# evolbioinfo/pastml

Measured on AMD Instinct MI355X. Metric: ACR nodes*states*chars/sec (full marginal pass: P(t) + bottom-up + top-down + posteriors), higher is better.
Workload: dtype f64; 1 GPU; BASELINE config 4 shard: balanced tree, 1048576 tips (2097151 nodes), k=64 states, F81, 32 characters per GPU (32 in total), marginal (BU+TD+posteriors); tips=1048576, nodes=2097151, states=64, chars_per_gpu=32, chars_total=32, substitution_model=F81, collective=local

## Files before the change

### pastml_amd/csrc/pml_kernels_f81.h

```cpp
#pragma once
#include "pml_device.h"
#include "pml_schedule.h"

typedef unsigned char pml_jt;

struct PmlTree {
    int N;
    int n_roots;
    const int* parent;
    const int* first_child;
    const int* n_children;
    const double* dist;
    const int* post_rank;
    const unsigned char* kind;
};

struct PmlCols {
    int k, ks, W;
    int no_wide_lean;
    const u64* masks;
    const u64* masks_init;
    const double* pi;
    const double* active;
};
// ... 2045 lines not shown
    double te[2][2], ts[2][2];
    u64 tw[2][2][Q];
#pragma unroll
    for (int j = 0; j < 2; ++j) {
        const int ch = fc + (j < nc ? j : 0);
        const int code = j < nc ? unit_code(u.packed, j) : 0;
        ce[j] = L.E[ch];
        lane_words_issue<G, R>(L, c, ch, cw[j]);
        cs[j] = L.S[ch];
        cbe[j] = code == 1 ? L.be[ch] : 0;
        if (code == 1) {
            node_load_vec<G, R>(L, c, L.bu, ch, vv[j]);
        } else {
#pragma unroll
            for (int r = 0; r < R; ++r) vv[j][r] = 0.0;
        }
        const int cfc = j == 0 ? cfc0 : cfc1;
#pragma unroll
        for (int q = 0; q < 2; ++q) {
            te[j][q] = 0.0;
            ts[j][q] = 0.0;
#pragma unroll
            for (int x = 0; x < Q; ++x) tw[j][q][x] = 0ull;
            if (code >= 2 && q < code - 1) {
                te[j][q] = L.E[cfc + q];
                ts[j][q] = L.S[cfc + q];
                lane_words_issue<G, R>(L, c, cfc + q, tw[j][q]);
            }
        }
    }
    double prod[R];
#pragma unroll
    for (int r = 0; r < R; ++r) prod[r] = po[r] * (ls * L.ipi_r[r]);
#pragma unroll
    for (int j = 0; j < 2; ++j) {
        if (j < nc) {
            const int ch = fc + j;
            const int code = unit_code(u.packed, j);
            const double e = ce[j];
            unsigned cb[Q];
            lane_words_bits<G, R>(L, c, cw[j], cb);
            double mb[R], tdc[R], pc[R], lsc;
            bits_to_vec<R>(cb, mb);
            i64 xe, le;
            if (code == 0) {
                f81_finish_child<G, R>(L, c, prod, pe, ch, e, cs[j], 0, mb, false, mb, tdc, xe, pc, lsc, le, -1);
            } else if (code == 1) {
                double v[R];
#pragma unroll
                for (int r = 0; r < R; ++r) v[r] = vv[j][r];
                f81_finish_child<G, R>(L, c, prod, pe, ch, e, cs[j], cbe[j], v, false, mb, tdc, xe, pc, lsc, le, -1);
                if (st.td != nullptr) {
                    node_store_vec<G, R>(L, c, L.td, ch, tdc);
                    if (L.g == 0) L.te[ch] = xe;
                }
            } else {
                double v[R];
#pragma unroll
                for (int r = 0; r < R; ++r) v[r] = mb[r];
                double amin = 1.0;
                i64 bec = 0;
                unsigned tb[2][Q];
#pragma unroll
                for (int q = 0; q < 2; ++q) {
                    lane_words_bits<G, R>(L, c, tw[j][q], tb[q]);
                    if (q < code - 1) {
                        const double ta = (1.0 - te[j][q]) * ts[j][q];
                        double tmsg[R];
                        bits_select_vec<R>(tb[q], ta, te[j][q], tmsg);
                        amin *= ta;
#pragma unroll
                        for (int r = 0; r < R; ++r) v[r] *= tmsg[r];
                    }
                }
                if (!(amin >= 0x1p-190)) bec = lazy_rescale<G, R>(v);
                f81_finish_child<G, R>(L, c, prod, pe, ch, e, cs[j], bec, v, false, mb, tdc, xe, pc, lsc, le, -1);
                double prod2[R];
#pragma unroll
                for (int r = 0; r < R; ++r) prod2[r] = pc[r] * (lsc * L.ipi_r[r]);
                const int cfc = j == 0 ? cfc0 : cfc1;
#pragma unroll
                for (int q = 0; q < 2; ++q) {
                    if (q < code - 1) {
                        double mt[R], tdt[R], pt[R], lt;
                        bits_to_vec<R>(tb[q], mt);
                        i64 xt, et;
                        f81_finish_child<G, R>(L, c, prod2, le, cfc + q, te[j][q], ts[j][q], 0, mt, false, mt, tdt, xt, pt, lt, et, -1);
                    }
                }
            }
        }
    }
}

template <int G, int R, bool LEAN = false, bool SHAPES = false>
__device__ __forceinline__ void td_f81_unit(const LaneCtx<G, R>& L, const PmlTree& t, const PmlCols& c,
                                            const PmlState& st, const UnitRegs& u) {
    if (LEAN && G < 8 && c.W == 1 && unit_is_lean(u.packed)) {
        const int key = u.packed & (15 | (63 << 8));
        const int key0 = __builtin_amdgcn_readfirstlane(key);
        if (SHAPES && __ballot(key != key0) == 0ull) {
            switch (key0) {
                case PML_SHAPE_KEY(2, 1, 1): td_f81_unit_lean<G, R, 1, 1>(L, t, c, st, u); break;
                case PML_SHAPE_KEY(2, 3, 3): td_f81_unit_lean<G, R, 3, 3>(L, t, c, st, u); break;
                case PML_SHAPE_KEY(2, 1, 0): td_f81_unit_lean<G, R, 1, 0>(L, t, c, st, u); break;
                case PML_SHAPE_KEY(2, 0, 1): td_f81_unit_lean<G, R, 0, 1>(L, t, c, st, u); break;
                case PML_SHAPE_KEY(2, 1, 3): td_f81_unit_lean<G, R, 1, 3>(L, t, c, st, u); break;
                case PML_SHAPE_KEY(2, 3, 1): td_f81_unit_lean<G, R, 3, 1>(L, t, c, st, u); break;
                case PML_SHAPE_KEY(2, 0, 3): td_f81_unit_lean<G, R, 0, 3>(L, t, c, st, u); break;
                case PML_SHAPE_KEY(2, 3, 0): td_f81_unit_lean<G, R, 3, 0>(L, t, c, st, u); break;
                default: td_f81_unit_lean<G, R>(L, t, c, st, u); break;
            }
        } else {
            td_f81_unit_lean<G, R>(L, t, c, st, u);
        }
        return;
    }
    if (SHAPES && LEAN && G >= 2 && G < 8 && c.W == 1 && !c.no_wide_lean) {
        const bool poly = unit_is_lean_poly(u.packed);
        if (__ballot(!poly) == 0ull) {
            td_f81_unit_lean_poly<G, R>(L, t, c, st, u);
            return;
        }
    }
    if constexpr (G >= 32) {
        if (LEAN && c.W > 1 && !c.no_wide_lean && unit_is_lean(u.packed)) {
            const int cfc0 = __shfl(u.cfc, L.group_base, 64), cfc1 = __shfl(u.cfc, L.group_base + Gather<G>::GC, 64);
            td_f81_unit_lean_w<G, R>(L, t, c, st, u, cfc0, cfc1);
            return;
        }
    }
    if (Gather<G>::enabled && c.W == 1 && unit_is_fast<G>(u.packed)) {
        td_f81_unit_fast<G, R>(L, t, c, st, u);
        return;
    }
    const int p = u.n;

    double prod[R];
    i64 pe;
    f81_parent_prod<G, R>(L, c, p, prod, pe);
    double P = 0.0;
    bool have_P = false;
    const int fc = u.fc;
    int nc = unit_nc(u.packed);
    if (nc == 15) nc = t.n_children[p];
    for (int j = 0; j < nc; ++j) {
        const int ch = fc + j;
        const ChildDesc cd = unit_child<G>(t, u, j, ch);
        const int kd = cd.kind;
        const int slot = j < 2 ? j : -1;
        if (kd == PML_KIND_TIP) {
            f81_finish_tip<G, R>(L, c, prod, pe, P, have_P, ch, slot);
            continue;
        }
        const double e = L.E[ch];
        double mb[R], v[R], tdc[R], po[R], ls;
        node_mask_vec<G, R>(L, c, ch, mb);
        i64 xe, le;
        if (kd == PML_KIND_STORED) {
            node_load_vec<G, R>(L, c, L.bu, ch, v);
            f81_finish_child<G, R>(L, c, prod, pe, ch, e, L.S[ch], L.be[ch], v, false, mb, tdc, xe, po, ls, le, slot);
            if (st.td != nullptr) {
                node_store_vec<G, R>(L, c, L.td, ch, tdc);
                if (L.g == 0) L.te[ch] = xe;
            }
        } else {
            i64 bec;
            f81_cherry_vector<G, R>(L, t, c, st, ch, v, bec, false, cd.tips_known, cd.fc2, cd.nc2);
            const double s_child = L.S[ch];
            f81_finish_child<G, R>(L, c, prod, pe, ch, e, s_child, bec, v, false, mb, tdc, xe, po, ls, le, slot);
            double prod2[R];
#pragma unroll
            for (int r = 0; r < R; ++r) prod2[r] = po[r] * (ls * L.ipi_r[r]);
            const i64 pe2 = le;
            double P2 = 0.0;
            bool have_P2 = false;
            const int fc2 = cd.tips_known ? cd.fc2 : t.first_child[ch];
            const int nc2 = cd.tips_known ? cd.nc2 : t.n_children[ch];
            for (int q = 0; q < nc2; ++q)
                f81_finish_tip<G, R>(L, c, prod2, pe2, P2, have_P2, fc2 + q, (j < 2 && q < 2) ? 2 + 2 * j + q : -1);
        }
    }
}

struct TdStage {
    double* rows;
    double* sum;
    i64* exp;
    int* id;
    int* tid;
    int* tst;
};
__host__ __device__ __forceinline__ int td_stage_doubles(int uw, int ks, bool scalars) {
    return uw * 2 * ks + (scalars ? uw * 12 : 0) + uw * 5;
}

template <int G, int R>
__device__ __forceinline__ void td_stage_flush(const LaneCtx<G, R>& L, const PmlCols& c, const TdStage& S, bool tips) {
    typedef double dbl2 __attribute__((ext_vector_type(2)));
    constexpr int UW = 64 / G;
    wave_sync_lds();
    const int lane = threadIdx.x & 63;
    const int ppr = c.ks >> 1;
    for (int p = lane; p < UW * 2 * ppr; p += 64) {
        const int slot = p / ppr, piece = p - slot * ppr;
        const int node = S.id[slot];
        if (node >= 0) {
            const dbl2 v = *reinterpret_cast<const dbl2*>(S.rows + slot * c.ks + 2 * piece);
            __builtin_nontemporal_store(v, reinterpret_cast<dbl2*>(L.post + (size_t)(unsigned)node * c.ks + 2 * piece));
        }
    }
    for (int p = lane; tips && p < UW * 4 * ppr; p += 64) {
        const int slot = p / ppr, piece = p - slot * ppr;
        const int node = S.tid[slot];
        if (node >= 0) {
            const int s = S.tst[slot];
            dbl2 v;
            v.x = s == 2 * piece ? 1.0 : 0.0;
            v.y = s == 2 * piece + 1 ? 1.0 : 0.0;
            __builtin_nontemporal_store(v, reinterpret_cast<dbl2*>(L.post + (size_t)(unsigned)node * c.ks + 2 * piece));
        }
    }
    if (S.sum != nullptr) {
        for (int e = lane; e < UW * 6; e += 64) {
            const int u = e / 6, j = e - u * 6;
            if (j >= 2 && !tips) continue;
            const int node = j < 2 ? S.id[u * 2 + j] : S.tid[u * 4 + j - 2];
            if (node >= 0) {
                L.lhsum[node] = S.sum[e];
                L.lhe[node] = S.exp[e];
            }
        }
    }
    wave_sync_lds();
    for (int e = lane; e < UW * 2; e += 64) S.id[e] = -1;
    for (int e = lane; tips && e < UW * 4; e += 64) S.tid[e] = -1;
    wave_sync_lds();
}

template <int G, int R>
__global__ void __launch_bounds__(PML_BLOCK)
td_f81_kernel(PmlTree t, PmlCols c, PmlState st, const PmlUnit* __restrict__ units, int n_level, int stage) {
    extern __shared__ double td_stage[];
    constexpr int UW = 64 / G;
    const int wave = threadIdx.x >> 6;
    const int sub = (threadIdx.x & 63) / G;
    LaneCtx<G, R> L;
    lane_ctx_init<G, R>(L, t, c, st);
    TdStage S = {nullptr, nullptr, nullptr, nullptr, nullptr, nullptr};
    const bool staged = G <= PML_TD_STAGE_MAX_G && (stage & 1) && (c.ks & 1) == 0;
    if (staged) {
        const bool scalars = (stage & 2) != 0;
        double* base = td_stage + wave * td_stage_doubles(UW, c.ks, scalars);
        S.rows = base;
        base += UW * 2 * c.ks;
        if (scalars) {
            S.sum = base;
            S.exp = reinterpret_cast<i64*>(base + UW * 6);
            base += UW * 12;
        }
        S.id = reinterpret_cast<int*>(base);
        S.tid = S.id + UW * 2;
        S.tst = S.tid + UW * 4;
        L.srow = S.rows + sub * 2 * c.ks;
        L.sid = S.id + sub * 2;
        L.stid = S.tid + sub * 4;
        L.stst = S.tst + sub * 4;
        if (scalars) {
            L.ssum = S.sum + sub * 6;
            L.sexp = S.exp + sub * 6;
        }
        for (int e = threadIdx.x & 63; e < UW * 2; e += 64) S.id[e] = -1;
        for (int e = threadIdx.x & 63; e < UW * 4; e += 64) S.tid[e] = -1;
        wave_sync_lds();
    }
    const int stride = gridDim.x * PML_WAVES_PER_BLOCK * UW;
    int idx = (blockIdx.x * PML_WAVES_PER_BLOCK + wave) * UW + sub;
    UnitRegs cur = load_unit<G>(units, idx < n_level ? idx : 0, L.g);
    for (int base = idx - sub; base < n_level; base += stride) {
        const int nxt_idx = idx + stride;
        const UnitRegs nxt = load_unit<G>(units, nxt_idx < n_level ? nxt_idx : 0, L.g);
        if (idx < n_level) td_f81_unit<G, R, true>(L, t, c, st, cur);
        if (staged) td_stage_flush<G, R>(L, c, S, (stage & 4) != 0);
        cur = nxt;
        idx = nxt_idx;
    }
}


template <int G, int R>
__device__ __forceinline__ void td_f81_super_tips(const LaneCtx<G, R>& L, const PmlCols& c, const double (&prod3)[R],
                                                  i64 le, int cfc, const TipLane& tl, int jx) {
    constexpr int GC = Gather<G>::GC;
    double P3 = 0.0;
    bool have_P3 = false;
#pragma unroll
    for (int q = 0; q < 2; ++q) {
        const int ts = L.group_base + jx * GC + q;
        f81_finish_tip_word<G, R>(L, c, prod3, le, P3, have_P3, cfc + q, __shfl(tl.mask, ts, 64), __shfl(tl.e, ts, 64),
                                  __shfl(tl.s, ts, 64));
    }
}

template <int G, int R, bool LANES>
__device__ __forceinline__ void td_f81_super_unit(const LaneCtx<G, R>& L, const PmlTree& t, const PmlCols& c,
                                                  const PmlState& st, const SuperRegs& s, int j, double* ps_row) {
    const u64 kbits = state_bits(c.k);
    const int ch = s.fc + j;
    const UnitRegs u = super_child<G>(s, j, L.g);
    double prod[R];
    i64 pe;
    f81_parent_prod<G, R>(L, c, s.n, prod, pe);
    const double e = L.E[ch];
    const double s_child = L.S[ch];
    const i64 bec = L.be[ch];
    BuLoads<R> ld;
    ld.own = L.mask[(unsigned)ch];
    f81_gather_issue<G, R>(L, u, ld.cl, ld.tl);
    f81_gather_finish<G, R>(L, ld.cl, ld.tl);
    ld.own &= kbits;
    const bool all_ones = __all(c.k == G * R && ld.own == kbits && ld.cl.mask == kbits);
    BuResult<R> v;
    CherryKeep<R> ck;
    if (all_ones) bu_f81_marg_body<G, R, false, true, true>(L, t, c, st, u, ld, &v, false, true, &ck);
    else bu_f81_marg_body<G, R, false, false, true>(L, t, c, st, u, ld, &v, false, true, &ck);
    double prod2[R];
    i64 pe2;
    {
        double mb[R], tdc[R], po[R], ls;
        const bool full = ld.own == kbits;
        if (!full) clean_word_to_vec<G, R>(L, c, ld.own, mb);
        i64 xe;
        f81_finish_child<G, R>(L, c, prod, pe, ch, e, s_child, bec, v.v, full, mb, tdc, xe, po, ls, pe2);
        if (st.td != nullptr) {
            node_store_vec<G, R>(L, c, L.td, ch, tdc);
            if (L.g == 0) L.te[ch] = xe;
        }
#pragma unroll
        for (int r = 0; r < R; ++r) prod2[r] = po[r] * (ls * L.ipi_r[r]);
    }
    constexpr int GC = Gather<G>::GC;
    const bool tip_lane = (L.g & ~(GC | 1)) == 0;
    const int tjx = (L.g / GC) & 1;
    bool lanes = LANES && c.W == 1 && !group_any<G>(tip_lane && __popcll(ld.tl.mask) != 1);
    double prod3[2][R], P3[2], ps = 0.0;
    i64 le3[2];
#pragma unroll
    for (int jx = 0; jx < 2; ++jx) {
        const int src = L.group_base + jx;
        const int cch = u.fc + jx;
        const double ce = __shfl(ld.cl.e, src, 64);
        const u64 word = __shfl(ld.cl.mask, src, 64);
        double mb[R], tdc[R], po[R], ls;
        const bool full = word == kbits;
        if (!full) clean_word_to_vec<G, R>(L, c, word, mb);
        i64 xe;
        f81_finish_child<G, R>(L, c, prod2, pe2, cch, ce, __shfl(ld.cl.s, src, 64), ck.e[jx], ck.v[jx], full, mb, tdc, xe, po,
                               ls, le3[jx]);
#pragma unroll
        for (int r = 0; r < R; ++r) prod3[jx][r] = po[r] * (ls * L.ipi_r[r]);
        if (!lanes) {
            td_f81_super_tips<G, R>(L, c, prod3[jx], le3[jx], __shfl(u.cfc, L.group_base + jx * GC, 64), ld.tl, jx);
            continue;
        }
        P3[jx] = pi_dot<G, R>(L, prod3[jx]);
#pragma unroll
        for (int r = 0; r < R; r += 2) {
            double2 t2;
            t2.x = prod3[jx][r];
            t2.y = prod3[jx][r + 1];
            *reinterpret_cast<double2*>(ps_row + L.st(r)) = t2;
        }
        wave_sync_lds();
        if (tip_lane && tjx == jx) ps = ps_row[__builtin_ctzll(ld.tl.mask)];
        wave_sync_lds();
    }
    if (!lanes) return;
    double lhs, lsum;
    bool ok;
    i64 le;
    f81_tip_closed_form(tjx ? P3[1] : P3[0], ps, ld.tl.e, ld.tl.s, tjx ? le3[1] : le3[0], lhs, ok, lsum, le);
    lanes = !isinf(P3[0]) && !isnan(P3[0]) && !isinf(P3[1]) && !isnan(P3[1]) && !group_any<G>(tip_lane && !ok);
    if (!lanes) {
#pragma unroll
        for (int jx = 0; jx < 2; ++jx)
            td_f81_super_tips<G, R>(L, c, prod3[jx], le3[jx], __shfl(u.cfc, L.group_base + jx * GC, 64), ld.tl, jx);
        return;
    }
    if (tip_lane) {
        const int tip = u.cfc + (L.g & 1);
        L.lhsum[tip] = lsum;
        L.lhe[tip] = le;
    }
    if (!L.implicit_tips) {
        const int ts = (int)__builtin_ctzll(ld.tl.mask | (1ull << 63));
#pragma unroll
        for (int q = 0; q < 4; ++q) {
            const int sq = __shfl(ts, L.group_base + (q >> 1) * GC + (q & 1), 64);
            double oh[R];
#pragma unroll
            for (int r = 0; r < R; ++r) oh[r] = L.st(r) == sq ? 1.0 : 0.0;
            node_store_vec_nt<G, R>(L, c, L.post, s.t0 + 4 * j + q, oh);
        }
    }
}

template <int G, int R, bool LANES>
__global__ void __launch_bounds__(PML_BLOCK)
td_f81_super_kernel(PmlTree t, PmlCols c, PmlState st, const PmlUnit* __restrict__ units, int n_level) {
    constexpr int UW = 64 / G;
    const int wave = threadIdx.x >> 6;
    const int sub = (threadIdx.x & 63) / G;
    __shared__ __attribute__((aligned(16))) double tip_rows[LANES ? PML_BLOCK * R : 2];
    double* const ps_row = LANES ? tip_rows + (wave * UW + sub) * (G * R) : nullptr;
    LaneCtx<G, R> L;
    lane_ctx_init<G, R>(L, t, c, st);
    const int n_units = 2 * n_level;
    const int stride = gridDim.x * PML_WAVES_PER_BLOCK * UW;
    int idx = (blockIdx.x * PML_WAVES_PER_BLOCK + wave) * UW + sub;
    SuperRegs cur = load_super(units, idx < n_units ? idx >> 1 : 0);
    for (int base = idx - sub; base < n_units; base += stride) {
        const int nxt_idx = idx + stride;
        const SuperRegs nxt = load_super(units, nxt_idx < n_units ? nxt_idx >> 1 : 0);
        if (idx < n_units) td_f81_super_unit<G, R, LANES>(L, t, c, st, cur, idx & 1, ps_row);
        cur = nxt;
        idx = nxt_idx;
    }
}

struct StackRegs {
    int n, fc, g0, g1;
};

__device__ __forceinline__ StackRegs load_stack(const PmlUnit* __restrict__ units, int idx) {
    const int4 h = *reinterpret_cast<const int4*>(units + idx);
    const int4 f = *reinterpret_cast<const int4*>(units[idx].cfc);
    StackRegs s;
    s.n = h.x;
    s.fc = h.y;
    s.g0 = f.x;
    s.g1 = f.y;
    return s;
}

__device__ __forceinline__ UnitRegs stack_child(const StackRegs& s, int j) {
    UnitRegs u;
    u.n = s.fc + j;
    u.fc = j ? s.g1 : s.g0;
    u.packed = PML_PACKED_TWO_STORED;
    u.cfc = u.cfc1 = u.cfc2 = u.cfc3 = 0;
    return u;
}

template <int G, int R>
__device__ __forceinline__ void stack_child_loads(const LaneCtx<G, R>& L, const PmlCols& c, int node, int first,
                                                  BuLoads<R>& ld) {
    const int ch = first + (L.g & 1);
    ld.cl.e = L.E[ch];
    ld.cl.s = L.S[ch];
    ld.cl.be = L.be[ch];
    ld.cl.mask = 0ull;
    ld.tl.e = ld.tl.s = ld.tl.a = 0.0;
    ld.tl.mask = 0ull;
    ld.own = L.mask[(unsigned)node];
    node_load_vec<G, R>(L, c, L.bu, first, ld.v0);
    node_load_vec<G, R>(L, c, L.bu, first + 1, ld.v1);
}

template <int G, int R>
__device__ __forceinline__ bool bu_f81_stack_unit(const LaneCtx<G, R>& L, const PmlTree& t, const PmlCols& c,
                                                  const PmlState& st, const StackRegs& s) {
    BuLoads<R> ld[2];
#pragma unroll
    for (int j = 0; j < 2; ++j) stack_child_loads<G, R>(L, c, s.fc + j, j ? s.g1 : s.g0, ld[j]);
    const double e_top = L.E[s.fc + (L.g & 1)];
    const u64 own = L.mask[(unsigned)s.n];
    BuResult<R> res[2];
#pragma unroll
    for (int j = 0; j < 2; ++j)
        if (!bu_f81_marg_body<G, R, true, false>(L, t, c, st, stack_child(s, j), ld[j], &res[j], false)) return false;
    BuLoads<R> top;
    top.cl.e = e_top;
    top.cl.s = (L.g & 1) ? res[1].s : res[0].s;
    top.cl.be = (L.g & 1) ? res[1].e : res[0].e;
    top.cl.mask = 0ull;
    top.tl.e = top.tl.s = top.tl.a = 0.0;
    top.tl.mask = 0ull;
    top.own = own;
#pragma unroll
    for (int r = 0; r < R; ++r) {
        top.v0[r] = res[0].v[r];
        top.v1[r] = res[1].v[r];
    }
    UnitRegs un;
    un.n = s.n;
    un.fc = s.fc;
    un.packed = PML_PACKED_TWO_STORED;
    un.cfc = un.cfc1 = un.cfc2 = un.cfc3 = 0;
    return bu_f81_marg_body<G, R, true, false>(L, t, c, st, un, top);
}

template <int G, int R>
__global__ void __launch_bounds__(PML_BLOCK) __attribute__((amdgpu_waves_per_eu(2, 2)))
bu_f81_stack_kernel(PmlTree t, PmlCols c, PmlState st, const PmlUnit* __restrict__ units, int n_level) {
    constexpr int UW = 64 / G;
    const int wave = threadIdx.x >> 6;
    const int sub = (threadIdx.x & 63) / G;
    LaneCtx<G, R> L;
    lane_ctx_init<G, R>(L, t, c, st);
    const int stride = gridDim.x * PML_WAVES_PER_BLOCK * UW;
    int idx = (blockIdx.x * PML_WAVES_PER_BLOCK + wave) * UW + sub;
    StackRegs cur = load_stack(units, idx < n_level ? idx : 0);
    for (int base = idx - sub; base < n_level; base += stride) {
        const int nxt_idx = idx + stride;
        const StackRegs nxt = load_stack(units, nxt_idx < n_level ? nxt_idx : 0);
        if (idx < n_level) {
            if (!bu_f81_stack_unit<G, R>(L, t, c, st, cur)) {
                bu_f81_unit_seq<G, R, false>(L, t, c, st, stack_child(cur, 0));
                bu_f81_unit_seq<G, R, false>(L, t, c, st, stack_child(cur, 1));
                __threadfence();
                UnitRegs un = stack_child(cur, 0);
                un.n = cur.n;
                un.fc = cur.fc;
                bu_f81_unit_seq<G, R, false>(L, t, c, st, un);
            }
        }
        cur = nxt;
        idx = nxt_idx;
    }
}

template <int G, int R>
__device__ __forceinline__ void td_f81_stack_unit(const LaneCtx<G, R>& L, const PmlTree& t, const PmlCols& c,
                                                  const PmlState& st, const StackRegs& s, int j) {
    const u64 kbits = state_bits(c.k);
    const int ch = s.fc + j;
    const int first = j ? s.g1 : s.g0;
    double prod[R];
    i64 pe;
    f81_parent_prod<G, R>(L, c, s.n, prod, pe);
    const double e = L.E[ch];
    const double s_child = L.S[ch];
    const i64 bec = L.be[ch];
    BuLoads<R> ld;
    stack_child_loads<G, R>(L, c, ch, first, ld);
    const u64 gmask = L.mask[(unsigned)(first + (L.g & 1))] & kbits;
    ld.own &= kbits;
    BuResult<R> v;
    double g0v[R], g1v[R];
#pragma unroll
    for (int r = 0; r < R; ++r) {
        g0v[r] = ld.v0[r];
        g1v[r] = ld.v1[r];
    }
    bu_f81_marg_body<G, R, true, false>(L, t, c, st, stack_child(s, j), ld, &v, false, true);
    double prod2[R];
    i64 pe2;
    {
        double mb[R], tdc[R], po[R], ls;
        const bool full = ld.own == kbits;
        if (!full) clean_word_to_vec<G, R>(L, c, ld.own, mb);
        i64 xe;
        f81_finish_child<G, R>(L, c, prod, pe, ch, e, s_child, bec, v.v, full, mb, tdc, xe, po, ls, pe2);
        if (st.td != nullptr) {
            node_store_vec<G, R>(L, c, L.td, ch, tdc);
            if (L.g == 0) L.te[ch] = xe;
        }
#pragma unroll
        for (int r = 0; r < R; ++r) prod2[r] = po[r] * (ls * L.ipi_r[r]);
    }
#pragma unroll
    for (int jx = 0; jx < 2; ++jx) {
        const int src = L.group_base + jx;
        const u64 word = __shfl(gmask, src, 64);
        double mb[R], tdc[R], po[R], ls;
        const bool full = word == kbits;
        if (!full) clean_word_to_vec<G, R>(L, c, word, mb);
        i64 xe, le;
        f81_finish_child<G, R>(L, c, prod2, pe2, first + jx, __shfl(ld.cl.e, src, 64), __shfl(ld.cl.s, src, 64),
                               __shfl(ld.cl.be, src, 64), jx ? g1v : g0v, full, mb, tdc, xe, po, ls, le);
        if (st.td != nullptr) {
            node_store_vec<G, R>(L, c, L.td, first + jx, tdc);
            if (L.g == 0) L.te[first + jx] = xe;
        }
    }
}

template <int G, int R>
__global__ void __launch_bounds__(PML_BLOCK)
td_f81_stack_kernel(PmlTree t, PmlCols c, PmlState st, const PmlUnit* __restrict__ units, int n_level) {
    constexpr int UW = 64 / G;
    const int wave = threadIdx.x >> 6;
    const int sub = (threadIdx.x & 63) / G;
    LaneCtx<G, R> L;
    lane_ctx_init<G, R>(L, t, c, st);
    const int n_units = 2 * n_level;
    const int stride = gridDim.x * PML_WAVES_PER_BLOCK * UW;
    int idx = (blockIdx.x * PML_WAVES_PER_BLOCK + wave) * UW + sub;
    StackRegs cur = load_stack(units, idx < n_units ? idx >> 1 : 0);
    for (int base = idx - sub; base < n_units; base += stride) {
        const int nxt_idx = idx + stride;
        const StackRegs nxt = load_stack(units, nxt_idx < n_units ? nxt_idx >> 1 : 0);
        if (idx < n_units) td_f81_stack_unit<G, R>(L, t, c, st, cur, idx & 1);
        cur = nxt;
        idx = nxt_idx;
    }
}

#define PML_SMALL_BLOCK 512

__device__ __forceinline__ double column_loglik(const PmlTree& t, const PmlCols& c, const PmlState& st, int col,
                                                int is_marginal) {
    const size_t colN = (size_t)col * t.N;
    double total = 0.0;
    for (int r = 0; r < t.n_roots; ++r) {
        const bool tip = t.n_children[r] == 0;
        const u64* m = c.masks + (colN + r) * c.W;
        double term;
        if (is_marginal) {
            term = 0.0;
            for (int s = 0; s < c.k; ++s) {
                const double b = tip ? (double)((m[s >> 6] >> (s & 63)) & 1ull) : st.bu[(colN + r) * c.ks + s];
                term += b * c.pi[(size_t)col * c.ks + s];
            }
        } else {
            term = -INFINITY;
            int arg = 0;
            for (int s = 0; s < c.k; ++s) {
                const double b = tip ? (double)((m[s >> 6] >> (s & 63)) & 1ull) : st.bu[(colN + r) * c.ks + s];
                const double v = b * c.pi[(size_t)col * c.ks + s];
                if (v > term) {
                    term = v;
                    arg = s;
                }
            }
            st.js[colN + r] = arg;
        }
        const double e2 = tip ? 0.0 : (double)st.be[colN + r];
        total += log(term) + e2 * 0.693147180559945309417232121458;
    }
    return total;
}

template <int G, int R, bool BU>
__device__ __forceinline__ void walk_levels(const LaneCtx<G, R>& L, const PmlTree& t, const PmlCols& c, const PmlState& st,
                                            const PmlUnit* __restrict__ units, const int* __restrict__ lv, int nl) {
    constexpr int UW = 64 / G;
    const int wave = threadIdx.x >> 6;
    const int n_waves = blockDim.x >> 6;
    const int sub = (threadIdx.x & 63) / G;
    const int first = wave * UW + sub;
    if (nl <= 0) return;
    int a = lv[0], b = lv[1];
    UnitRegs nxt = load_unit<G>(units, first < b - a ? a + first : a, L.g);
    for (int l = 0; l < nl; ++l) {
        const int n_level = b - a;
        const UnitRegs cur = nxt;
        int a2 = a, b2 = a;
        if (l + 1 < nl) {
            a2 = lv[l + 1];
            b2 = lv[l + 2];
            nxt = load_unit<G>(units, first < b2 - a2 ? a2 + first : a2, L.g);
        }
        if (first < n_level) {
            if (BU) bu_f81_unit<G, R, false, true, true>(L, t, c, st, cur);
            else td_f81_unit<G, R, true, true>(L, t, c, st, cur);
        }
        for (int base = wave * UW + n_waves * UW; base < n_level; base += n_waves * UW) {
            const int idx = base + sub;
            if (idx < n_level) {
                if (BU) bu_f81_unit<G, R, false, true, true>(L, t, c, st, load_unit<G>(units, a + idx, L.g));
                else td_f81_unit<G, R, true, true>(L, t, c, st, load_unit<G>(units, a + idx, L.g));
            }
        }
        __syncthreads();
        a = a2;
        b = b2;
    }
}


template <int G, int R>
__global__ void __launch_bounds__(PML_SMALL_BLOCK)
bu_f81_small_kernel(PmlTree t, PmlCols c, PmlState st, const double* __restrict__ mu, const double* __restrict__ sf,
                    const double* __restrict__ tau, const double* __restrict__ tauf, int do_prep,
                    const PmlUnit* __restrict__ units, const int* __restrict__ level_offsets, int n_levels,
                    double* __restrict__ loglik, u64* __restrict__ err_out, int reset_err,
                    u64* __restrict__ done_state, u64* done_flag) {
    const int col = blockIdx.y;
    if (!column_active(c, col)) {
        if (threadIdx.x == 0 && done_flag != nullptr) {
            if (atomicAdd(&done_state[0], 1ull) == (u64)gridDim.y - 1ull) {
                done_state[0] = 0ull;
                const u64 generation = done_state[1] + 1ull;
                done_state[1] = generation;
                __threadfence_system();
                *reinterpret_cast<volatile u64*>(done_flag) = generation;
            }
        }
        return;
    }
    if (reset_err) {
        if (threadIdx.x == 0) st.err[col] = ~0ull;
        __syncthreads();
    }
    if (do_prep) {
        const size_t colN = (size_t)col * t.N;
        const double m = mu[col], s = sf[col], ta = tau[col], tf = tauf[col];
        for (int n = threadIdx.x; n < t.N; n += blockDim.x) {
            const double tt = (t.dist[n] + ta) * tf * s;
            st.E[colN + n] = isinf(m) ? 0.0 : exp(-m * tt);
            if (t.n_children[n] == 0) {
                double acc = 0.0;
                for (int w = 0; w < c.W; ++w) {
                    u64 word = c.masks[(colN + n) * c.W + w];
                    while (word) {
                        const int b = __builtin_ctzll(word);
                        acc += c.pi[(size_t)col * c.ks + w * 64 + b];
                        word &= word - 1ull;
                    }
                }
                st.S[colN + n] = acc;
            }
        }
        __syncthreads();
    }
    LaneCtx<G, R> L;
    lane_ctx_init<G, R>(L, t, c, st);
    walk_levels<G, R, true>(L, t, c, st, units, level_offsets, n_levels);
// ... 117 lines not shown
```

### pastml_amd/csrc/pml_launch_f81_super.hip

```cpp
#include "pml_launch.h"

template <int G, int R>
static void launch_super_f81(pml_ctx* ctx, bool bottom_up) {
    const PmlTree t = tree_of(ctx, true);
    const PmlCols c = cols_of(ctx, bottom_up);
    const PmlState st = state_of(ctx);
    const int upb = PML_WAVES_PER_BLOCK * (64 / G);
    dim3 grid(grid_for(ctx, bottom_up ? ctx->sup.n : 2 * ctx->sup.n, upb, ctx->C, bottom_up), ctx->C), block(PML_BLOCK);
    if (bottom_up)
        hipLaunchKernelGGL((bu_f81_super_kernel<G, R>), grid, block, 0, ctx->stream, t, c, st, ctx->sup.d_units, ctx->sup.n);
    else if (ctx->tune.on(T_NO_TIP_LANES))
        hipLaunchKernelGGL((td_f81_super_kernel<G, R, false>), grid, block, 0, ctx->stream, t, c, st, ctx->sup.d_units, ctx->sup.n);
    else
        hipLaunchKernelGGL((td_f81_super_kernel<G, R, true>), grid, block, 0, ctx->stream, t, c, st, ctx->sup.d_units, ctx->sup.n);
}

template <int G, int R>
static void launch_stack_f81(pml_ctx* ctx, bool bottom_up, int a, int n) {
    const PmlTree t = tree_of(ctx, true);
    const PmlCols c = cols_of(ctx, bottom_up);
    const PmlState st = state_of(ctx);
    const int upb = PML_WAVES_PER_BLOCK * (64 / G);
    dim3 grid(grid_for(ctx, bottom_up ? n : 2 * n, upb, ctx->C), ctx->C), block(PML_BLOCK);
    if (bottom_up)
        hipLaunchKernelGGL((bu_f81_stack_kernel<G, R>), grid, block, 0, ctx->stream, t, c, st, ctx->sup.d_stack_bu + a, n);
    else
        hipLaunchKernelGGL((td_f81_stack_kernel<G, R>), grid, block, 0, ctx->stream, t, c, st, ctx->sup.d_stack_td + a, n);
}

int dispatch_super_f81(pml_ctx* ctx, bool bottom_up) {
    if (ctx->sup.n <= 0) return PML_OK;
    int g, r;
    super_shape(ctx, bottom_up, g, r);
#define X(G_, R_)                                   \
    if (g == G_ && r == R_) {                       \
        launch_super_f81<G_, R_>(ctx, bottom_up);   \
        HIP_TRY(hipGetLastError());                 \
        return PML_OK;                              \
    }
    PML_SUPER_CASES(X)
#undef X
    return fail(PML_ERR_UNSUPPORTED, "no two-level F81 kernel for G=%d R=%d", g, r);
}

int dispatch_stack_f81(pml_ctx* ctx, bool bottom_up, int level) {
    const std::vector<int>& off = bottom_up ? ctx->sup.stack_bu_offsets : ctx->sup.stack_td_offsets;
    if (ctx->sup.n_stack == 0 || level + 1 >= (int)off.size()) return PML_OK;
    const int a = off[level], n = off[level + 1] - a;
    if (n <= 0) return PML_OK;
    int g, r;
    super_shape(ctx, bottom_up, g, r);
#define X(G_, R_)                                         \
    if (g == G_ && r == R_) {                             \
        launch_stack_f81<G_, R_>(ctx, bottom_up, a, n);   \
        HIP_TRY(hipGetLastError());                       \
        return PML_OK;                                    \
    }
    PML_SUPER_CASES(X)
#undef X
    return fail(PML_ERR_UNSUPPORTED, "no stacked F81 kernel for G=%d R=%d", g, r);
}
```

### pastml_amd/csrc/pml_schedule.h

```cpp
#pragma once
#include <cstdlib>
#include <string>
#include <vector>

#define PML_KIND_TIP 0
#define PML_KIND_CHERRY 1
#define PML_KIND_STORED 2

struct __attribute__((aligned(32))) PmlUnit {
    int n, fc, packed, pad;
    int cfc[4];
};

#define PML_PACKED_TWO_STORED ((1 << 11) | (1 << 8) | (3 << 4) | 2)

#define PML_TUNABLES(X)                                                                                              \
    X(GRID_CAP, 0, 0) X(SMALL_MANY_NODES, 0, 0) X(BLOCK_MAX_WORK, 0, 0)    \
    X(NO_MFMA, 1, 0) X(NO_EIGEN_FUSED, 1, 0) X(NO_HKY_FUSED, 1, 0)      \
    X(BLOCK_THREADS, 0, 0) X(EIG_BLOCKS, 0, 0) X(NO_EIGEN_GEMM, 1, 0) X(NO_EIGEN_JOINT_VALU, 1, 0) X(EIGJ_BLOCKS, 0, 0) \
    X(EIGJ_TIP_BLOCKS, 0, 0) X(EIGJ_ONE_TIPS_KERNEL, 1, 0) X(EIGJ_TIER_THIN, 0, 1) X(EIGJ_TIER_DEPTH, 0, 1)            \
    X(NO_EIGJ_TIERS, 1, 1) X(NO_BT_TIERS, 1, 1) X(NO_SHAPE_SORT, 1, 1) X(NO_SUPER, 1, 1) X(SUPER_MIN, 0, 1)            \
    X(STACK_MIN, 0, 1) X(NO_STACK, 1, 1) X(DEBUG, 1, 0) X(BLOCK_NODES, 0, 1) X(BLOCK_MAX_STORED, 0, 1)                 \
    X(BLOCK_HEIGHT_CAP, 0, 1) X(SMALL_MAX_NODES, 0, 1) X(F81_R, 0, 1) X(F81_TD_R, 0, 1) X(NO_GRAPH, 1, 1)              \
    X(NARROW_UNITS, 0, 0) X(NO_EIGG_TIERS, 1, 0) X(NO_SPIN_WAIT, 1, 0)   \
    X(PIJ_STAGE_ROWS, 0, 0) X(PIJ_BLOCKS, 0, 0) X(NO_HEIGHT_ORDER, 1, 1) X(NO_TD_TAIL, 1, 0) X(NO_PIJ_VALU, 1, 0) X(PIJ_VALU, 1, 0) X(NO_PIJ_WIDE, 1, 0) X(NO_EIGJ_PIPE, 1, 0) \
    X(THIN_UNITS, 0, 1) X(THIN_BYTES, 0, 1) X(THIN_BLOCK_NODES, 0, 1) X(NO_THIN, 1, 0) X(NO_THIN_WIDE, 1, 0) X(BU_WIDE, 0, 1) X(SORT_LEVELS, 0, 1) X(NO_WIDE_LEAN, 1, 0) X(SHAPE_ORDER, 0, 1) \
    X(PARS_MAX_COLS, 0, 0) X(PARS_THIN, 0, 0) X(COMPRESS_MAX_COLS, 0, 0) X(COMPRESS_PLAIN_ATOMICS, 1, 0) \
    X(PIJ_WINDOW, 0, 0) X(NO_KEEP_TIP_ROWS, 1, 0) X(NO_TIP_LANES, 1, 0)
enum PmlTunable {
#define X(name, flag, tree) T_##name,
    PML_TUNABLES(X)
#undef X
    T_COUNT
};
static const char* const kTunableName[T_COUNT] = {
#define X(name, flag, tree) #name,
    PML_TUNABLES(X)
#undef X
};
static const bool kTunableFlag[T_COUNT] = {
#define X(name, flag, tree) flag != 0,
    PML_TUNABLES(X)
#undef X
};
static const bool kTunableTree[T_COUNT] = {
#define X(name, flag, tree) tree != 0,
    PML_TUNABLES(X)
#undef X
};
struct PmlTune {
    long long val[T_COUNT];
    bool has[T_COUNT];
    PmlTune() {
        for (int i = 0; i < T_COUNT; ++i) {
            const std::string var = std::string("PASTML_HIP_") + kTunableName[i];
            const char* e = getenv(var.c_str());
            has[i] = e != nullptr;
            val[i] = e ? atoll(e) : 0;
        }
    }
    bool on(int i) const { return has[i]; }
    long long get(int i, long long dflt) const { return has[i] ? val[i] : dflt; }
};

struct PmlBlockSchedule {
    bool ok = false;
    int n_blocks = 0;
    long long steps = 0;
    PmlUnit *d_bu_units = nullptr, *d_td_units = nullptr;
    int *d_bu_start = nullptr, *d_bu_levels = nullptr, *d_bu_lv = nullptr;
    int *d_td_start = nullptr, *d_td_levels = nullptr, *d_td_lv = nullptr;
    PmlUnit *d_top_bu_units = nullptr, *d_top_td_units = nullptr;
    int *d_top_bu_offsets = nullptr, *d_top_td_offsets = nullptr;
    std::vector<int> top_bu_offsets, top_td_offsets;
    std::vector<char> top_bu_vec;
};
struct PmlThinSchedule {
    bool ok = false;
    int floor_level = 0;
    int top_level = 0;
    struct Tier { int first_block, n_blocks; };
    std::vector<Tier> tiers;
    PmlUnit* d_units = nullptr;
    int *d_start = nullptr, *d_levels = nullptr, *d_lv = nullptr;
};
struct PmlDeepSchedule {
    bool ok = false;
    int first_depth = 0, n_blocks = 0;
    PmlUnit* d_units = nullptr;
    int *d_start = nullptr, *d_levels = nullptr, *d_lv = nullptr;
};
struct PmlSuperSchedule {
    bool ok = false;
    int n = 0;
    PmlUnit* d_units = nullptr;
    PmlUnit* d_child_units = nullptr;
    PmlUnit *d_bu_units_r = nullptr, *d_td_units_r = nullptr;
    PmlUnit *d_bu_units_rs = nullptr, *d_td_units_rs = nullptr;
    int n_child_units = 0;
    int n_stack = 0;
    PmlUnit *d_stack_bu = nullptr, *d_stack_td = nullptr, *d_stack_children = nullptr;
    std::vector<int> stack_bu_offsets, stack_td_offsets;
    int *d_bu_offsets_r = nullptr, *d_td_offsets_r = nullptr;
    std::vector<int> bu_offsets_r, td_offsets_r;
    std::vector<char> bu_level_vec_r;
};
struct PmlEigenTiers {
    bool ok = false;
    int first_level = 0;
    int top_level = 0;
    struct Tier { int first_block, n_blocks, depth; };
    std::vector<Tier> tiers;
    PmlUnit* d_units = nullptr;
    int *d_lv = nullptr, *d_start = nullptr;
    int* d_nodes = nullptr;
    int widest = 0;
};
struct PmlBacktraceTiers {
    bool ok = false;
    int first_depth = 0;
    struct Tier { int first_block, n_blocks, depth; };
    std::vector<Tier> tiers;
    int *d_nodes = nullptr, *d_lv = nullptr, *d_start = nullptr;
};

struct PmlTreeArrays {
    int n_nodes, n_roots, n_bu_levels, n_td_levels;
    const int *parent, *first_child, *n_children, *bu_offsets, *bu_order, *td_offsets, *td_parent_offsets, *td_parents,
        *post_rank;
    const double* dist;
};

struct PmlNumbering {
    std::vector<int> old_of_new, new_of_old;
    std::vector<int> parent, first_child, n_children, bu_order, td_parents, post_rank;
    std::vector<double> dist;
};

struct PmlForest {
    bool fuse = true;
    int N = 0, n_roots = 0, n_internal = 0;
    std::vector<int> parent, first_child, n_children;
    std::vector<int> bu_offsets, td_offsets, td_parent_offsets;
    std::vector<unsigned char> kind;
    std::vector<int> fh;
    std::vector<int> order_f;
    std::vector<int> bu_offsets_f;
    std::vector<int> tdp;
    std::vector<int> td_parent_offsets_f;
    bool shape_ordered = false;
    bool polytomies = false;
    bool balanced_parts = false;
    int max_h() const { return (int)bu_offsets_f.size() - 1; }
    int n_stored() const { return bu_offsets_f.empty() ? 0 : bu_offsets_f.back(); }
};

struct PmlLevelTable {
    std::vector<int> list, start, levels, lv;
    template <class F>
    void add_runs(const int* mem, size_t count, F level) {
        start.push_back((int)lv.size());
        int nl = 0;
        for (size_t q = 0; q < count; ++q) {
            if (q == 0 || level(mem[q]) != level(mem[q - 1])) {
                lv.push_back((int)list.size());
                ++nl;
            }
            list.push_back(mem[q]);
        }
        lv.push_back((int)list.size());
        levels.push_back(nl);
    }
    template <class F>
    void add_cells(const int* mem, size_t count, F level, int first, int n) {
        start.push_back((int)lv.size());
        size_t q = 0;
        for (int d = 0; d < n; ++d) {
            lv.push_back((int)list.size());
            for (; q < count && level(mem[q]) == first + d; ++q) list.push_back(mem[q]);
        }
        lv.push_back((int)list.size());
        levels.push_back(n);
    }
};

struct PmlTreePlan {
    std::vector<int> tips, cherries;
    std::vector<PmlUnit> bu_units_f, td_units_f, bu_units, cherry_units;
    bool shape_sort = false;
    std::vector<PmlUnit> bu_units_fs, td_units_fs;
    std::vector<char> bu_level_vec_f, bu_level_vec;
    std::vector<int> td_cherry_prefix;
    bool small = false;
    struct { PmlEigenTiers s; PmlLevelTable t; std::vector<PmlUnit> units; } eig;
    struct { PmlBacktraceTiers s; PmlLevelTable t; } bt;
    struct {
        PmlSuperSchedule s;
        bool lists = false;
        std::vector<PmlUnit> units, child_units, bu_units_r, td_units_r, bu_units_rs, td_units_rs, stack_bu, stack_td,
            stack_children;
    } sup;
    struct { PmlBlockSchedule s; PmlLevelTable bu, td; std::vector<PmlUnit> bu_units, td_units, top_bu_units, top_td_units; } blocks;
};

struct PmlThinPlan {
    PmlThinSchedule thin;
    PmlDeepSchedule deep;
    PmlLevelTable bu, td;
    std::vector<PmlUnit> bu_units, td_units;
};

enum SweepKind {
    SW_BU_MARG, SW_BU_JOINT, SW_TD, SW_ROOTS, SW_BU_MARG_FUSED, SW_TD_FUSED, SW_BU_CHERRIES,
    SW_BU_MARG_FUSED_NOVEC,
    SW_BU_JOINT_NOVEC,
    SW_BU_JOINT_FUSED, SW_BU_JOINT_FUSED_NOVEC,
    SW_BU_CHERRIES_JOINT
};
enum PmlEigenFamily { EIG_JOINT, EIG_GEMM, EIG_FUSED };
enum PmlOp {
    OP_RESET_ERR, OP_PREP, OP_LOGLIK,
    OP_LEVEL,
    OP_LEVELS,
    OP_BLOCKS,
    OP_SUPER, OP_STACK,
    OP_ROOTS,
    OP_EIG_TIPS, OP_EIG_LEVEL, OP_EIG_NARROW, OP_EIG_TIER,
    OP_BT_NARROW, OP_BT_TIER, OP_BT_LEVEL,
    OP_COUNT
};
enum PmlList {
    L_NONE, L_BU_FUSED, L_BU_FUSED_SORTED, L_TD_FUSED, L_TD_FUSED_SORTED, L_BU_PLAIN, L_TD_PLAIN, L_CHERRIES, L_TOP_BU, L_TOP_TD,
    L_REST_BU, L_REST_BU_SORTED, L_REST_TD, L_REST_TD_SORTED, L_CHILD_UNITS, L_STACK_CHILDREN,
    L_IDS,
    L_COUNT
};
enum PmlBranch {
    BU_ONE_LAUNCH, BU_BLOCKS, BU_SUPER, BU_THIN, BU_FUSED, BU_FUSED_JOINT, BU_EIGJ_TIERS, BU_EIGJ, BU_GEMM_TIERS, BU_GEMM,
    BU_EIG_FUSED, BU_PLAIN, TD_ONE_LAUNCH, TD_BLOCKS, TD_SUPER, TD_GEMM, TD_EIG_FUSED, TD_DEEP, TD_LEVELS, BT_TIERS, BT_LEVELS,
    PML_BRANCH_COUNT
};
#define PML_NO_BRACKET 255
struct PmlLaunch {
    unsigned char op, list, kind;
    unsigned char bracket;
    unsigned char branch;
    bool signal;
    bool cherries;
    int first, count;
    int arg;
};
struct PmlSweepOutcome {
    int n_signals = 0;
    bool final_signals = false;
    bool has_params = false;
    bool fused_joint = false;
    void then(const PmlSweepOutcome& next) {
        n_signals += next.n_signals;
        final_signals = next.final_signals;
        has_params = has_params || next.has_params;
        fused_joint = fused_joint || next.fused_joint;
    }
};
struct PmlSweepTraits {
    bool f81, eigen_fused, eigen_gemm, eigen_joint_valu, hky_fused, wide_states;
    int k, W, C, sched_cols, n_roots, n_cherries;
    bool has_init, fuse;
    int Gf, Gt;
    bool bu_wide_lanes, level_lists_sorted;
    bool single_launch, blocks, super, thin, deep;
    int narrow_units;
    bool no_td_tail, no_eigg_tiers, no_spin_wait;
    int waves, eig_nb;
};
struct PmlSchedules {
    const PmlBlockSchedule* blocks;
    const PmlThinSchedule* thin;
    const PmlDeepSchedule* deep;
    const PmlSuperSchedule* sup;
    const PmlEigenTiers* eig;
    const PmlBacktraceTiers* bt;
    const std::vector<char>*bu_level_vec_f, *bu_level_vec;
    const std::vector<int>* td_cherry_prefix;
};

#define PML_PLAN __attribute__((visibility("hidden")))
PML_PLAN std::string pml_check_tree(const PmlTreeArrays& t);
PML_PLAN PmlForest pml_plan_forest(PmlTreeArrays& t, const PmlTune& tune, bool fuse, PmlNumbering& num);
PML_PLAN PmlTreePlan pml_plan_tree(const PmlForest& f, const PmlTreeArrays& t, const PmlTune& tune);
PML_PLAN PmlThinPlan pml_plan_thin_ends(const PmlForest& f, const PmlTune& tune, int thin);
PML_PLAN std::vector<PmlLaunch> pml_plan_bottom_up(const PmlForest& f, const PmlSchedules& s, const PmlSweepTraits& t, bool is_marginal);
PML_PLAN std::vector<PmlLaunch> pml_plan_top_down(const PmlForest& f, const PmlSchedules& s, const PmlSweepTraits& t, bool wants_signal);
PML_PLAN std::vector<PmlLaunch> pml_plan_backtrace(const PmlForest& f, const PmlSchedules& s, const PmlSweepTraits& t, int* head);
PML_PLAN PmlSweepOutcome pml_plan_outcome(const std::vector<PmlLaunch>& plan);
```

Before: 580.3 billion node*state*char/s.

## Software-pipeline top-down super-unit loads one unit ahead in F81 kernel

Splits the top-down two-level F81 kernel into a load-issue phase and a compute phase. It double-buffers the per-unit loads (parent posterior, likelihood sums, child scalars, masks and child gathers), so the next unit's global loads are in flight while the current unit is computed. It also sets a waves-per-EU attribute for the pipelined R=8 variant and passes the pipe flag to the grid sizing. The extra live registers for the second buffer may lower occupancy, and a tunable flag can turn the pipelined path off.

Measured after the change: 609.2 billion node*state*char/s, median of 6. +5.0%, better.

```diff
diff --git a/pastml_amd/csrc/pml_kernels_f81.h b/pastml_amd/csrc/pml_kernels_f81.h
--- a/pastml_amd/csrc/pml_kernels_f81.h
+++ b/pastml_amd/csrc/pml_kernels_f81.h
@@ -2371,21 +2371,60 @@
     }
 }
 
-template <int G, int R, bool LANES>
+template <int R>
+struct TdSuperLoads {
+    double po[R];
+    double ls;
+    i64 pe;
+    double e, s;
+    i64 be;
+    u64 own;
+    ChildLane cl;
+    TipLane tl;
+};
+
+template <int G, int R>
+__device__ __forceinline__ void td_f81_super_issue(const LaneCtx<G, R>& L, const PmlCols& c, const SuperRegs& s, int j,
+                                                   TdSuperLoads<R>& ld) {
+    const int ch = s.fc + j;
+    node_load_vec<G, R>(L, c, L.post, s.n, ld.po);
+    ld.ls = L.lhsum[s.n];
+    ld.pe = L.lhe[s.n];
+    ld.e = L.E[ch];
+    ld.s = L.S[ch];
+    ld.be = L.be[ch];
+    ld.own = L.mask[(unsigned)ch];
+    f81_gather_issue<G, R>(L, super_child<G>(s, j, L.g), ld.cl, ld.tl);
+}
+
+template <int R>
+__device__ __forceinline__ void td_super_loads_arrived(TdSuperLoads<R>& ld) {
+#pragma unroll
+    for (int r = 0; r < R; ++r) asm volatile("" : "+v"(ld.po[r]));
+    asm volatile("" : "+v"(ld.ls), "+v"(ld.pe), "+v"(ld.e), "+v"(ld.s), "+v"(ld.be), "+v"(ld.own));
+    asm volatile("" : "+v"(ld.cl.e), "+v"(ld.cl.s), "+v"(ld.cl.mask), "+v"(ld.cl.be), "+v"(ld.tl.e), "+v"(ld.tl.s),
+                      "+v"(ld.tl.mask));
+}
+
+template <int G, int R, bool LANES, bool PIPE>
 __device__ __forceinline__ void td_f81_super_unit(const LaneCtx<G, R>& L, const PmlTree& t, const PmlCols& c,
-                                                  const PmlState& st, const SuperRegs& s, int j, double* ps_row) {
+                                                  const PmlState& st, const SuperRegs& s, int j, TdSuperLoads<R>& in,
+                                                  double* ps_row) {
+    if (PIPE) td_super_loads_arrived<R>(in);
     const u64 kbits = state_bits(c.k);
     const int ch = s.fc + j;
     const UnitRegs u = super_child<G>(s, j, L.g);
     double prod[R];
-    i64 pe;
-    f81_parent_prod<G, R>(L, c, s.n, prod, pe);
-    const double e = L.E[ch];
-    const double s_child = L.S[ch];
-    const i64 bec = L.be[ch];
+    const i64 pe = in.pe;
+#pragma unroll
+    for (int r = 0; r < R; ++r) prod[r] = in.po[r] * (in.ls * L.ipi_r[r]);
+    const double e = in.e;
+    const double s_child = in.s;
+    const i64 bec = in.be;
     BuLoads<R> ld;
-    ld.own = L.mask[(unsigned)ch];
-    f81_gather_issue<G, R>(L, u, ld.cl, ld.tl);
+    ld.own = in.own;
+    ld.cl = in.cl;
+    ld.tl = in.tl;
     f81_gather_finish<G, R>(L, ld.cl, ld.tl);
     ld.own &= kbits;
     const bool all_ones = __all(c.k == G * R && ld.own == kbits && ld.cl.mask == kbits);
@@ -2474,8 +2513,9 @@
     }
 }
 
-template <int G, int R, bool LANES>
+template <int G, int R, bool LANES, bool PIPE>
 __global__ void __launch_bounds__(PML_BLOCK)
+    __attribute__((amdgpu_waves_per_eu(PIPE && R == 8 ? 2 : 1, PIPE && R == 8 ? 2 : 8)))
 td_f81_super_kernel(PmlTree t, PmlCols c, PmlState st, const PmlUnit* __restrict__ units, int n_level) {
     constexpr int UW = 64 / G;
     const int wave = threadIdx.x >> 6;
@@ -2487,13 +2527,47 @@
     const int n_units = 2 * n_level;
     const int stride = gridDim.x * PML_WAVES_PER_BLOCK * UW;
     int idx = (blockIdx.x * PML_WAVES_PER_BLOCK + wave) * UW + sub;
-    SuperRegs cur = load_super(units, idx < n_units ? idx >> 1 : 0);
-    for (int base = idx - sub; base < n_units; base += stride) {
-        const int nxt_idx = idx + stride;
-        const SuperRegs nxt = load_super(units, nxt_idx < n_units ? nxt_idx >> 1 : 0);
-        if (idx < n_units) td_f81_super_unit<G, R, LANES>(L, t, c, st, cur, idx & 1, ps_row);
-        cur = nxt;
-        idx = nxt_idx;
+    const int j = idx & 1;
+    int base = idx - sub;
+    if (!PIPE) {
+        SuperRegs cur = load_super(units, idx < n_units ? idx >> 1 : 0);
+        for (; base < n_units; base += stride) {
+            const int nxt_idx = idx + stride;
+            const SuperRegs nxt = load_super(units, nxt_idx < n_units ? nxt_idx >> 1 : 0);
+            if (idx < n_units) {
+                TdSuperLoads<R> ld;
+                td_f81_super_issue<G, R>(L, c, cur, j, ld);
+                td_f81_super_unit<G, R, LANES, false>(L, t, c, st, cur, j, ld, ps_row);
+            }
+            cur = nxt;
+            idx = nxt_idx;
+        }
+        return;
+    }
+    SuperRegs ua = load_super(units, idx < n_units ? idx >> 1 : 0);
+    SuperRegs ub = load_super(units, idx + stride < n_units ? (idx + stride) >> 1 : 0);
+    TdSuperLoads<R> la, lb;
+    td_f81_super_issue<G, R>(L, c, ua, j, la);
+    while (base < n_units) {
+        {
+            const int i2 = idx + 2 * stride;
+            const SuperRegs un = load_super(units, i2 < n_units ? i2 >> 1 : 0);
+            td_f81_super_issue<G, R>(L, c, ub, j, lb);
+            if (idx < n_units) td_f81_super_unit<G, R, LANES, true>(L, t, c, st, ua, j, la, ps_row);
+            ua = un;
+            idx += stride;
+            base += stride;
+        }
+        if (base >= n_units) break;
+        {
+            const int i2 = idx + 2 * stride;
+            const SuperRegs un = load_super(units, i2 < n_units ? i2 >> 1 : 0);
+            td_f81_super_issue<G, R>(L, c, ua, j, la);
+            if (idx < n_units) td_f81_super_unit<G, R, LANES, true>(L, t, c, st, ub, j, lb, ps_row);
+            ub = un;
+            idx += stride;
+            base += stride;
+        }
     }
 }
 
diff --git a/pastml_amd/csrc/pml_launch_f81_super.hip b/pastml_amd/csrc/pml_launch_f81_super.hip
--- a/pastml_amd/csrc/pml_launch_f81_super.hip
+++ b/pastml_amd/csrc/pml_launch_f81_super.hip
@@ -1,4 +1,10 @@
 #include "pml_launch.h"
+
+template <int G, int R, bool LANES, bool PIPE>
+static void launch_td_super_f81(pml_ctx* ctx, dim3 grid, const PmlTree& t, const PmlCols& c, const PmlState& st) {
+    hipLaunchKernelGGL((td_f81_super_kernel<G, R, LANES, PIPE>), grid, dim3(PML_BLOCK), 0, ctx->stream, t, c, st, ctx->sup.d_units,
+                       ctx->sup.n);
+}
 
 template <int G, int R>
 static void launch_super_f81(pml_ctx* ctx, bool bottom_up) {
@@ -6,13 +12,19 @@
     const PmlCols c = cols_of(ctx, bottom_up);
     const PmlState st = state_of(ctx);
     const int upb = PML_WAVES_PER_BLOCK * (64 / G);
-    dim3 grid(grid_for(ctx, bottom_up ? ctx->sup.n : 2 * ctx->sup.n, upb, ctx->C, bottom_up), ctx->C), block(PML_BLOCK);
+    const bool pipe = bottom_up || !ctx->tune.on(T_NO_TD_SUPER_PIPE);
+    dim3 grid(grid_for(ctx, bottom_up ? ctx->sup.n : 2 * ctx->sup.n, upb, ctx->C, pipe), ctx->C), block(PML_BLOCK);
+    const bool lanes = !ctx->tune.on(T_NO_TIP_LANES);
     if (bottom_up)
         hipLaunchKernelGGL((bu_f81_super_kernel<G, R>), grid, block, 0, ctx->stream, t, c, st, ctx->sup.d_units, ctx->sup.n);
-    else if (ctx->tune.on(T_NO_TIP_LANES))
-        hipLaunchKernelGGL((td_f81_super_kernel<G, R, false>), grid, block, 0, ctx->stream, t, c, st, ctx->sup.d_units, ctx->sup.n);
+    else if (pipe && lanes)
+        launch_td_super_f81<G, R, true, true>(ctx, grid, t, c, st);
+    else if (pipe)
+        launch_td_super_f81<G, R, false, true>(ctx, grid, t, c, st);
+    else if (lanes)
+        launch_td_super_f81<G, R, true, false>(ctx, grid, t, c, st);
     else
-        hipLaunchKernelGGL((td_f81_super_kernel<G, R, true>), grid, block, 0, ctx->stream, t, c, st, ctx->sup.d_units, ctx->sup.n);
+        launch_td_super_f81<G, R, false, false>(ctx, grid, t, c, st);
 }
 
 template <int G, int R>
diff --git a/pastml_amd/csrc/pml_schedule.h b/pastml_amd/csrc/pml_schedule.h
--- a/pastml_amd/csrc/pml_schedule.h
+++ b/pastml_amd/csrc/pml_schedule.h
@@ -26,7 +26,7 @@
     X(PIJ_STAGE_ROWS, 0, 0) X(PIJ_BLOCKS, 0, 0) X(NO_HEIGHT_ORDER, 1, 1) X(NO_TD_TAIL, 1, 0) X(NO_PIJ_VALU, 1, 0) X(PIJ_VALU, 1, 0) X(NO_PIJ_WIDE, 1, 0) X(NO_EIGJ_PIPE, 1, 0) \
     X(THIN_UNITS, 0, 1) X(THIN_BYTES, 0, 1) X(THIN_BLOCK_NODES, 0, 1) X(NO_THIN, 1, 0) X(NO_THIN_WIDE, 1, 0) X(BU_WIDE, 0, 1) X(SORT_LEVELS, 0, 1) X(NO_WIDE_LEAN, 1, 0) X(SHAPE_ORDER, 0, 1) \
     X(PARS_MAX_COLS, 0, 0) X(PARS_THIN, 0, 0) X(COMPRESS_MAX_COLS, 0, 0) X(COMPRESS_PLAIN_ATOMICS, 1, 0) \
-    X(PIJ_WINDOW, 0, 0) X(NO_KEEP_TIP_ROWS, 1, 0) X(NO_TIP_LANES, 1, 0)
+    X(PIJ_WINDOW, 0, 0) X(NO_KEEP_TIP_ROWS, 1, 0) X(NO_TIP_LANES, 1, 0) X(NO_TD_SUPER_PIPE, 1, 0)
 enum PmlTunable {
 #define X(name, flag, tree) T_##name,
     PML_TUNABLES(X)
```
